# epfl-lts2/pygsp

Hardware: AMD Instinct MI355X
Metric: filtered-vertices/sec (N·Nsig·K/s) + achieved HBM GB/s vs roofline, 1M-vertex K=30 (higher is better)
Workload: dtype f64

## Files before the change

pygsp_amd/csrc/gspx_ctx.hip.h:

```cpp
#pragma once

struct Options {
  int64_t kernel = 0;
  int64_t vec = 0;
  int64_t rows_per_wave = 0;
  int64_t narrow_g_log2 = -1;
  int64_t waves_per_block = 4;
  int64_t calib_mix = 0;
  int64_t graph_launch = 2;
  int64_t tile_gather = 1;
  int64_t tile_workgroups = 0;
  int64_t knn_f32 = 1;
  int64_t tile_pad = 1;
  int64_t tile_min_row = 16;
  int64_t staged_copy = 1;
  int64_t staged_copy_min_mb = 32;
  int64_t copy_threads = 0;
  int64_t tile_regroup = 1;
  int64_t tile_lg = 0;
  int64_t edge_vertex_walk = 1;
  int64_t fuse_input = 1;
  int64_t tile_nt = -1;
  int64_t synthesis = 0;
  int64_t alternate_sweep = 1;
  int64_t xcd_remap = 1;
  int64_t combine = 0;
  int64_t ws_limit_mb = 65536;
  int64_t max_batch = 0;
  int64_t gather_rccl = 1;
  int64_t lds_pad_kb = 0;
  int64_t host_pipeline = 1;
  int64_t host_batch = 0;
  int64_t host_edge = 0;
  int64_t host_threads = 0;
  int64_t streamed_alloc = 1;
};

struct gspx_ctx {
  int device = 0;
  int cu_count = 256;
  hipStream_t stream = nullptr;
  Options opt;
  DevMem ws_t;
  DevMem ws_r;
  DevMem ws_w;
  DevMem io_x, io_y;
  DevMem ws_spec;
  DevMem ws_sq, ws_sqp;
  HostPipe* pipe = nullptr;
  CopyStage* copy = nullptr;
  bool counted = false;
  std::mutex comms_mu;
  std::vector<struct gspx_comm*> comms;
  hipEvent_t ev[4] = {nullptr, nullptr, nullptr, nullptr};
  std::vector<hipEvent_t> ev_pool;
  double timing[5] = {0, 0, 0, 0, 0};
  bool capturing = false;
  std::vector<unsigned char> seen_key;
  std::vector<unsigned char> graph_key;
  hipGraphExec_t graph_exec = nullptr;
};

static std::atomic<int> g_live_ctx[64];

static void replay_reset(gspx_ctx* ctx) {
  if (!ctx) return;
  ctx->seen_key.clear();
  ctx->graph_key.clear();
  if (ctx->graph_exec) {
    (void)hipGraphExecDestroy(ctx->graph_exec);
    ctx->graph_exec = nullptr;
  }
}

static int finish_timed(gspx_ctx* ctx, double* kernel_ms) {
  HIPCHK(hipGetLastError());
  HIPCHK(hipStreamSynchronize(ctx->stream));
  float f = 0;
  HIPCHK(hipEventElapsedTime(&f, ctx->ev[0], ctx->ev[1]));
  if (kernel_ms) *kernel_ms = f;
  return GSPX_OK;
}

struct gspx_buf {
  gspx_ctx* ctx = nullptr;
  DevMem mem;
  int64_t bytes = 0;
};

static std::atomic<uint64_t> g_generation{1};

struct gspx_graph {
  gspx_ctx* ctx = nullptr;
  const uint64_t generation = g_generation.fetch_add(1);
  int64_t N = 0;
  int dtype = GSPX_F64;
  bool from_w = false;
  int64_t nnz_l = 0;
  DevMem lptr, lcol, lval, dw;
  int64_t nnz_int = 0;
  DevMem rptr, rcol, rval, fval, coff;
// ... 88 lines not shown
    delete ctx;
    return set_err(GSPX_ERR_HIP, "hipStreamCreate failed: %s", hipGetErrorString(e));
  }
  for (int i = 0; i < 4; ++i) {
    e = hipEventCreate(&ctx->ev[i]);
    if (e != hipSuccess) {
      delete ctx;
      return set_err(GSPX_ERR_HIP, "hipEventCreate failed: %s", hipGetErrorString(e));
    }
  }
  *out = ctx;
  return GSPX_OK;
}

static void comm_invalidate_all(gspx_ctx* ctx);

extern "C" int gspx_ctx_destroy(gspx_ctx* ctx) {
  replay_reset(ctx);
  if (!ctx) return GSPX_OK;
  if (ctx->counted) g_live_ctx[ctx->device & 63].fetch_sub(1);
  comm_invalidate_all(ctx);
  if (ctx->graph_exec) {
    (void)hipGraphExecDestroy(ctx->graph_exec);
    ctx->graph_exec = nullptr;
  }
  (void)hipSetDevice(ctx->device);
  if (ctx->stream) (void)hipStreamSynchronize(ctx->stream);
  for (int i = 0; i < 4; ++i)
    if (ctx->ev[i]) (void)hipEventDestroy(ctx->ev[i]);
  for (hipEvent_t e : ctx->ev_pool) (void)hipEventDestroy(e);
  ctx->ws_t.release();
  ctx->ws_r.release();
  ctx->ws_w.release();
  ctx->io_x.release();
  ctx->io_y.release();
  ctx->ws_spec.release();
  ctx->ws_sq.release();
  ctx->ws_sqp.release();
  if (ctx->pipe) {
    ctx->pipe->destroy();
    delete ctx->pipe;
    ctx->pipe = nullptr;
  }
  if (ctx->copy) {
    ctx->copy->destroy();
    delete ctx->copy;
    ctx->copy = nullptr;
  }
  if (ctx->stream) (void)hipStreamDestroy(ctx->stream);
  delete ctx;
  return GSPX_OK;
}

extern "C" int gspx_ctx_sync(gspx_ctx* ctx) {
  if (!ctx) return set_err(GSPX_ERR_INVALID, "null ctx");
  HIPCHK(hipSetDevice(ctx->device));
  HIPCHK(hipStreamSynchronize(ctx->stream));
  return GSPX_OK;
}

struct OptionDef {
  const char* key;
  int64_t Options::*slot;
  bool (*ok)(int64_t);
  const char* refusal;
};
static const OptionDef OPTION_TABLE[] = {
    {"kernel", &Options::kernel, [](int64_t v) { return v == 0 || v == 1 || v == 2 || v == 5; },
     "kernel must be 0 (auto), 1 (panel), 2 (narrow) or 5 (LDS-staged)"},
    {"vec", &Options::vec, [](int64_t v) { return v == 0 || v == 1 || v == 2 || v == 4; }, "vec must be 0, 1, 2 or 4"},
    {"rows_per_wave", &Options::rows_per_wave, [](int64_t v) { return v >= 0 && v <= 1024; },
     "rows_per_wave must be in [0, 1024] (0 = auto)"},
    {"narrow_g_log2", &Options::narrow_g_log2, [](int64_t v) { return v >= -1 && v <= 6; },
     "narrow_g_log2 must be in [-1, 6] (-1 = auto)"},
    {"waves_per_block", &Options::waves_per_block, [](int64_t v) { return v == 4 || v == 8 || v == 16; },
     "waves_per_block must be 4, 8 or 16"},
    {"alternate_sweep", &Options::alternate_sweep, nullptr, nullptr},
    {"synthesis", &Options::synthesis, nullptr, nullptr},
    {"tile_gather", &Options::tile_gather, nullptr, nullptr},
    {"graph_launch", &Options::graph_launch, nullptr, nullptr},
    {"tile_workgroups", &Options::tile_workgroups, nullptr, nullptr},
    {"tile_lg", &Options::tile_lg, nullptr, nullptr},
    {"tile_regroup", &Options::tile_regroup, nullptr, nullptr},
    {"staged_copy", &Options::staged_copy, nullptr, nullptr},
    {"staged_copy_min_mb", &Options::staged_copy_min_mb, nullptr, nullptr},
    {"copy_threads", &Options::copy_threads, nullptr, nullptr},
    {"tile_min_row", &Options::tile_min_row, nullptr, nullptr},
    {"tile_pad", &Options::tile_pad, nullptr, nullptr},
    {"knn_f32", &Options::knn_f32, nullptr, nullptr},
    {"tile_nt", &Options::tile_nt, nullptr, nullptr},
    {"fuse_input", &Options::fuse_input, nullptr, nullptr},
    {"edge_vertex_walk", &Options::edge_vertex_walk, nullptr, nullptr},
    {"xcd_remap", &Options::xcd_remap, nullptr, nullptr},
    {"combine", &Options::combine, nullptr, nullptr},
    {"ws_limit_mb", &Options::ws_limit_mb, nullptr, nullptr},
    {"max_batch", &Options::max_batch, nullptr, nullptr},
    {"gather_rccl", &Options::gather_rccl, nullptr, nullptr},
    {"lds_pad_kb", &Options::lds_pad_kb, nullptr, nullptr},
    {"host_pipeline", &Options::host_pipeline, nullptr, nullptr},
    {"host_batch", &Options::host_batch, nullptr, nullptr},
    {"host_edge", &Options::host_edge, nullptr, nullptr},
    {"host_threads", &Options::host_threads, nullptr, nullptr},
    {"streamed_alloc", &Options::streamed_alloc, nullptr, nullptr},
};

static const OptionDef* find_option(const char* key) {
  if (key)
    for (const OptionDef& d : OPTION_TABLE)
      if (!strcmp(key, d.key)) return &d;
  set_err(GSPX_ERR_INVALID, "unknown option '%s'", key ? key : "(null)");
  return nullptr;
}

extern "C" int gspx_ctx_set_option(gspx_ctx* ctx, const char* key, int64_t value) {
  replay_reset(ctx);
  if (!ctx) return set_err(GSPX_ERR_INVALID, "null ctx");
  const OptionDef* d = find_option(key);
  if (!d) return GSPX_ERR_INVALID;
  if (d->ok && !d->ok(value)) return set_err(GSPX_ERR_INVALID, "%s", d->refusal);
  ctx->opt.*d->slot = value;
  if (d->slot == &Options::streamed_alloc) {
    const bool on = value != 0;
    (void)hipSetDevice(ctx->device);
    for (DevMem* m : {&ctx->ws_t, &ctx->ws_r}) {
      if (!on && m->va_size) {
        (void)hipStreamSynchronize(ctx->stream);
        m->release();
      }
      m->streamed = on;
    }
  }
  return GSPX_OK;
}

extern "C" int gspx_ctx_get_option(gspx_ctx* ctx, const char* key, int64_t* value) {
  if (!ctx || !value) return set_err(GSPX_ERR_INVALID, "null argument");
  if (key && !strcmp(key, "retired_va_mb")) {
    *value = (int64_t)(g_retired_va_bytes.load() >> 20);
    return GSPX_OK;
  }
  const OptionDef* d = find_option(key);
  if (!d) return GSPX_ERR_INVALID;
  *value = ctx->opt.*d->slot;
  return GSPX_OK;
}

extern "C" int gspx_buf_alloc(gspx_ctx* ctx, int64_t bytes, gspx_buf** out) {
  if (!ctx || !out || bytes < 0) return set_err(GSPX_ERR_INVALID, "gspx_buf_alloc: bad argument");
  *out = nullptr;
  HIPCHK(hipSetDevice(ctx->device));
  gspx_buf* b = new gspx_buf();
  b->ctx = ctx;
  b->bytes = bytes;
  int rc = b->mem.alloc((size_t)bytes);
  if (rc != GSPX_OK) {
    delete b;
    return rc;
  }
  *out = b;
  return GSPX_OK;
}

extern "C" int gspx_buf_free(gspx_buf* b) {
  if (!b) return GSPX_OK;
  (void)hipSetDevice(b->ctx->device);
  (void)hipStreamSynchronize(b->ctx->stream);
// ... 144 lines not shown
```

pygsp_amd/csrc/gspx_poly.hip.h:

```cpp
#pragma once

struct PlanStep {
  double scale = 1.0, gamma = -1.0;
  int flush = 0;
  int final = 0;
  std::vector<double> w;
};

static void make_plan_fused(int nf, int M, const std::vector<double>& cp, bool acc_existing,
                            bool final_to_y, std::vector<PlanStep>& plan) {
  const int K = M - 1;
  plan.assign((size_t)K, PlanStep());
  int covered = -1;
  bool first = !acc_existing;
  for (int k = 1; k <= K; ++k) {
    PlanStep& st = plan[(size_t)k - 1];
    st.scale = (k == 1) ? 0.5 : 1.0;
    st.gamma = (k == 1) ? 0.0 : -1.0;
    st.w.assign((size_t)nf * 3, 0.0);
    const bool must = (k == K) || (k >= 2 && (k - 2) > covered);
    if (!must) continue;
    st.flush = first ? 1 : 2;
    first = false;
    st.final = (k == K && final_to_y) ? 1 : 0;
// ... 250 lines not shown
}
static size_t sqnorm_parts(const gspx_ctx* ctx, int N, unsigned w) {
  return (size_t)sqnorm_gx(ctx, N, w) * SQ_PASS * w;
}

template <typename T>
static int launch_combine_sqnorm(gspx_ctx* ctx, const T* slots, int nslots, size_t slot_stride, unsigned pitch, int N,
                                 unsigned w, const SqNorms& sq, hipStream_t st) {
  const size_t lds = (size_t)nslots * 64 * sizeof(double);
  const int cwl = sqnorm_cwl(w);
  const dim3 grid((unsigned)sqnorm_gx(ctx, N, w), (w + (1u << cwl) - 1) >> cwl);
  for (int f0 = 0; f0 < sq.nf; f0 += SQ_PASS) {
    const int here = std::min(SQ_PASS, sq.nf - f0);
    const int fb = here <= 8 ? 2 : here <= 32 ? 8 : 32;
    typedef void (*kern_t)(const T*, int, size_t, u32, int, int, int, const double*, int, double*);
    const kern_t kern = fb == 2 ? k_combine_sqnorm<T, 2> : fb == 8 ? k_combine_sqnorm<T, 8> : k_combine_sqnorm<T, 32>;
    if (lds > ((size_t)64 << 10))
      HIPCHK(hipFuncSetAttribute((const void*)kern, hipFuncAttributeMaxDynamicSharedMemorySize, (int)lds));
    hipLaunchKernelGGL(kern, grid, dim3(256), lds, st, slots, nslots, slot_stride, (u32)pitch, N, (int)w, cwl,
                       sq.cf + f0, sq.ldc, sq.part);
    const int64_t n = (int64_t)here * w;
    hipLaunchKernelGGL(k_sqnorm_reduce, dim3((unsigned)((n + 255) / 256)), dim3(256), 0, st, sq.part, (int)grid.x,
                       4 * fb, here, (int)w, sq.out + (size_t)f0 * sq.ldo, sq.ldo);
  }
  return GSPX_OK;
}

template <typename T> static bool tile_geometry(const gspx_graph* g, const Options& opt, unsigned ld) {
  constexpr int TVEC = 16 / (int)sizeof(T);
  const size_t U = (size_t)g->N * ld;
  return opt.tile_gather && g->gt_rows == GSPX_TILE_BR && (size_t)ld * sizeof(T) >= (size_t)opt.tile_min_row &&
         (ld % TVEC) == 0 && U * sizeof(T) < ((size_t)1 << 31) && (size_t)g->nnz_int * sizeof(T) < ((size_t)1 << 31);
}
template <typename T>
static bool tile_usable(const gspx_graph* g, const Options& opt, unsigned ld, const T* y, unsigned ldy) {
  constexpr int TVEC = 16 / (int)sizeof(T);
  return tile_geometry<T>(g, opt, ld) && (ldy % TVEC) == 0 && (((uintptr_t)y / sizeof(T)) % TVEC) == 0;
}
template <typename T>
static int launch_step_tile(gspx_graph* g, const Options& opt, TileArgs<T> t, unsigned ld, hipStream_t st,
                            const T* vals = nullptr) {
  const size_t rowb = (size_t)ld * sizeof(T);
  int lg = rowb <= 16 ? 1 : rowb <= 32 ? 2 : rowb <= 64 ? 4 : rowb <= 128 ? 8 : 16;
  if (opt.tile_lg == 8 || opt.tile_lg == 4 || opt.tile_lg == 2) lg = rowb <= 128 ? std::max(lg, (int)opt.tile_lg) : 16;
  const bool narrow = lg < 16;
  const int ncol = narrow ? 1 : (int)((rowb + 255) / 256);
  const int flavour = t.old_rows ? 1 : t.nin > 0 ? 2 : 0;
  typedef void (*kern_t)(const TileArgs<T>);
  static const kern_t wide[3][3] = {
      {k_step_tile<T, 0>, k_step_tile<T, 1>, k_step_tile<T, 2>},
      {k_step_tile<T, 0, 16, true>, k_step_tile<T, 1, 16, true>, k_step_tile<T, 2, 16, true>},
      {k_step_tile<T, 0, 16, false, true>, k_step_tile<T, 1, 16, false, true>, k_step_tile<T, 2, 16, false, true>}};
  static const kern_t slim[3][4] = {
      {k_step_tile<T, 1, 1, false, false, 64>, k_step_tile<T, 1, 2, false, false, 128>,
       k_step_tile<T, 1, 4, false, false, 256>, k_step_tile<T, 1, 8>},
      {k_step_tile<T, 1, 1, true, false, 64>, k_step_tile<T, 1, 2, true, false, 128>,
       k_step_tile<T, 1, 4, true, false, 256>, k_step_tile<T, 1, 8, true>},
      {k_step_tile<T, 1, 1, false, true, 64>, k_step_tile<T, 1, 2, false, true, 128>,
       k_step_tile<T, 1, 4, false, true, 256>, k_step_tile<T, 1, 8, false, true>}};
  kern_t kern = narrow ? slim[flavour][lg == 1 ? 0 : lg == 2 ? 1 : lg == 4 ? 2 : 3] : wide[flavour][ncol <= 2 ? ncol : 0];
  unsigned threads = narrow ? 64u * (unsigned)lg : 512u;
  bool mix = false;
  if (opt.calib_mix && !narrow && flavour == 0) {
    static const kern_t mixk[2][3] = {
        {k_step_tile<T, 0, 16, false, false, 512, 16, 1>, k_step_tile<T, 1, 16, false, false, 512, 16, 1>,
         k_step_tile<T, 2, 16, false, false, 512, 16, 1>},
        {k_step_tile<T, 0, 16, false, false, 512, 16, 2>, k_step_tile<T, 1, 16, false, false, 512, 16, 2>,
         k_step_tile<T, 2, 16, false, false, 512, 16, 2>}};
    kern = mixk[opt.calib_mix == 2 ? 1 : 0][ncol <= 2 ? ncol : 0];
    mix = true;
  }
  const int pieces = (int)(rowb / 16);
  if (opt.tile_regroup && ncol == 1 && flavour != 1 && pieces < lg && !mix) {
#define GSPX_CL(LG_, CL_, NT_) \
  (flavour == 2 ? (kern_t)k_step_tile<T, 1, LG_, false, true, NT_, CL_> : (kern_t)k_step_tile<T, 1, LG_, false, false, NT_, CL_>)
    kern_t k2 = nullptr;
    unsigned nt2 = 0;
    if (lg == 4 && pieces == 3) k2 = GSPX_CL(4, 3, 192), nt2 = 192;
    else if (lg == 8 && pieces == 5) k2 = GSPX_CL(8, 5, 320), nt2 = 320;
    else if (lg == 16 && pieces == 10) k2 = GSPX_CL(16, 10, 320), nt2 = 320;
#undef GSPX_CL
    if (k2) kern = k2, threads = nt2;
  }
  size_t lds = g->gt_lds;
  if (lg < 8)
    lds = std::min(lds, (size_t)GSPX_TILE_MAXN1 * 16 * lg + (((size_t)g->gt_entmax * sizeof(T) + 15) & ~(size_t)15) +
                            (((size_t)g->gt_entmax + 15) & ~(size_t)15) + 64);
  if (lg < 8) lds = (lds + 2047) & ~(size_t)2047;
  int per_cu = 2;
  {
    struct Known { size_t attr = 0; std::map<size_t, int> fit; };
    static std::map<std::pair<const void*, int>, Known> known;
    static std::mutex lds_mu;
    std::lock_guard<std::mutex> lock(lds_mu);
    Known& k = known[std::make_pair((const void*)kern, g->ctx->device)];
    if (k.attr < lds) {
      HIPCHK(hipFuncSetAttribute((const void*)kern, hipFuncAttributeMaxDynamicSharedMemorySize, (int)lds));
      k.attr = lds;
    }
    if (lg < 8) {
      auto it = k.fit.find(lds);
      if (it == k.fit.end()) {
        int fit = 2;
        HIPCHK(hipOccupancyMaxActiveBlocksPerMultiprocessor(&fit, (const void*)kern, (int)threads, lds));
        it = k.fit.emplace(lds, std::max(2, std::min(fit, 16))).first;
      }
      per_cu = it->second;
    }
  }
  t.rowptr = g->rptr.as<int>();
  t.col = g->rcol.as<int>();
  t.val = vals ? vals : g->fval.as<T>();
  t.hdr = g->gt_hdr.as<int>();
  if (!t.s1rows) t.s1rows = g->gt_s1rows.as<int>();
  t.lidx = g->gt_lidx.as<unsigned char>();
  t.N = (int)g->N;
  t.ld = ld;
  t.panel_bytes = (unsigned)((size_t)g->N * ld * sizeof(T));
  t.val_bytes = (unsigned)((size_t)g->nnz_int * sizeof(T));
  t.lidx_bytes = (unsigned)((size_t)g->nnz_int);
  t.nb = g->gt_nb;
  t.ncol = ncol;
  t.per_xcd = (t.nb + 7) / 8;
  t.lds_bytes = (int)lds;
  unsigned nwg = (unsigned)std::max<int64_t>(8, ((int64_t)per_cu * g->ctx->cu_count) / 8 * 8);
  if (opt.tile_workgroups > 0)
    nwg = (unsigned)std::max<int64_t>(8, std::min<int64_t>(opt.tile_workgroups, 1 << 20) / 8 * 8);
  nwg = std::min(nwg, 8u * (unsigned)std::max(t.per_xcd, 1));
  t.nt = opt.tile_nt >= 0 ? (int)opt.tile_nt : ((size_t)g->N * ld * sizeof(T) >= ((size_t)192 << 20) ? 5 : 0);
  hipLaunchKernelGGL(kern, dim3(nwg), dim3(threads), lds, st, t);
  return GSPX_OK;
}

template <typename T>
static int prepare_coff(gspx_graph* g, const Shape& shape, unsigned ld, hipStream_t st) {
  if (shape.kernel == 5 && g->coff_ldb != ld * (unsigned)sizeof(T)) {
    CHK(g->coff.ensure(((size_t)g->nnz_int + 64) * sizeof(unsigned)));
    const int nb = std::max(1, (int)((g->N + 255) / 256));
    hipLaunchKernelGGL((k_coff<T>), dim3(nb), dim3(256), 0, st, g->rptr.as<int>(), g->rcol.as<int>(), (int)g->N,
                       ld * (unsigned)sizeof(T), g->coff.as<unsigned>());
    g->coff_ldb = ld * (unsigned)sizeof(T);
  }
  return GSPX_OK;
}

template <typename T> static int vec_cap(int v, unsigned ld, const T* p) {
  while (v > 1 && ((ld % v) != 0 || (((uintptr_t)p / sizeof(T)) % v) != 0)) v /= 2;
  return v;
}

struct WorkPanels {
  bool tile_direct, padded;
  unsigned ldw;
};
template <typename T>
static WorkPanels work_panels(const gspx_graph* g, const Options& opt, bool tiles, size_t planes, unsigned ld,
                              const T* y, unsigned ldy) {
  constexpr unsigned TVEC = 16 / (unsigned)sizeof(T);
  const unsigned ldp = (ld + TVEC - 1) / TVEC * TVEC;
  auto window = [&](unsigned w) { return planes * (size_t)g->N * w * sizeof(T) < ((size_t)1 << 31); };
  const bool pad_pays = opt.tile_pad == 2 || ld >= 2 ||
                        (size_t)g->nnz_int * (sizeof(T) + 4) >= ((size_t)20 << 20);
  WorkPanels p;
  p.tile_direct = tiles && tile_usable<T>(g, opt, ld, y, ldy) && window(ld);
  p.padded = !p.tile_direct && tiles && opt.tile_pad && pad_pays && tile_geometry<T>(g, opt, ldp) && window(ldp);
  p.ldw = p.padded ? ldp : ld;
  return p;
}

template <typename T>
static StepArgs<T> step_base(const gspx_graph* g, unsigned ld, T* y, unsigned ldy) {
  StepArgs<T> a{};
  a.rowptr = g->rptr.as<int>();
  a.col = g->rcol.as<int>();
  a.val = g->fval.as<T>();
  a.N = (int)g->N;
  a.ld = ld;
  a.curbytes = (u32)((size_t)g->N * ld * sizeof(T));
  a.y = y;
  a.ldy = ldy;
  a.perm = g->has_perm ? g->perm.as<int>() : nullptr;
  return a;
}

static int batch_events(gspx_ctx* ctx, size_t& ev_idx, hipEvent_t ev[4]) {
  for (int i = 0; i < 4; ++i) ev[i] = pool_event(ctx, ++ev_idx);
  if (!ev[0] || !ev[1] || !ev[2] || !ev[3]) return set_err(GSPX_ERR_HIP, "hipEventCreate failed");
  HIPCHK(hipEventRecord(ev[0], ctx->stream));
  return GSPX_OK;
}

// ... 249 lines not shown
      continue;
    }
    a.wts = ctx->ws_w.as<T>() + (size_t)k * nf;
    a.final = (k == 0) ? 1 : 0;
    a.flush = 0;
    if (k == K) {
      a.cur = S;
      a.old = S;
      a.out = B[k & 1];
      a.scale = T(0);
      a.gamma = T(0);
    } else {
      a.cur = B[(k + 1) & 1];
      a.out = B[k & 1];
      const bool has_b2 = (k + 2 <= K);
      a.old = has_b2 ? B[k & 1] : a.cur;
      a.gamma = has_b2 ? T(-1) : T(0);
      a.scale = (k == 0) ? T(0.5) : T(1);
    }
    a.reverse = (opt.alternate_sweep && (k & 1)) ? 1 : 0;
    launch_step<T>(a, shape, opt, st, g->coff.as<unsigned>());
  }
  HIPCHK(hipEventRecord(ev[2], st));
  if (padded) {
    const unsigned nbp = (unsigned)std::min<size_t>(((size_t)N * ld + 255) / 256, 65536);
    hipLaunchKernelGGL((k_permute_out_pad<T>), dim3(nbp), dim3(256), 0, st, B[0], ldw, y, ldy, ld, N, perm);
  }
  HIPCHK(hipEventRecord(ev[3], st));
  HIPCHK(hipGetLastError());
  return GSPX_OK;
}

template <typename T>
static int run_program_batch(gspx_graph* g, int S, const double* sc, const double* be, const double* ga, bool old_is_x,
                             const T* x, unsigned ldx, T* y, unsigned ldy, unsigned ld, size_t& ev_idx) {
  gspx_ctx* ctx = g->ctx;
  Options opt = ctx->opt;
  hipStream_t st = ctx->stream;
  const int N = (int)g->N;
  const size_t U = (size_t)N * ld;
  const Shape shape = choose_shape(opt, sizeof(T), ld, vec_cap(4, ldy, y));
  const int* perm = g->has_perm ? g->perm.as<int>() : nullptr;

  const T hw[3] = {T(1), T(0), T(0)};
  CHK(ctx->ws_w.ensure(sizeof(hw) + 64));
  HIPCHK(hipMemcpyAsync(ctx->ws_w.p, hw, sizeof(hw), hipMemcpyHostToDevice, st));
  HIPCHK(hipStreamSynchronize(st));
  CHK(ctx->ws_t.ensure((old_is_x ? 3 : 2) * U * sizeof(T) + 256));
  T* X = ctx->ws_t.as<T>();
  T* H[2] = {X + U, old_is_x ? X + 2 * U : X};

  hipEvent_t ev[4];
  CHK(batch_events(ctx, ev_idx, ev));
  launch_permute_in<T>(x, ldx, X, ld, N, perm, vec_cap(shape.vec, ldx, x), st);
  HIPCHK(hipEventRecord(ev[1], st));

  CHK(prepare_coff<T>(g, shape, ld, st));
  StepArgs<T> a = step_base<T>(g, ld, y, ldy);
  a.nf = 1;
  a.racc = H[0];
  a.wts = ctx->ws_w.as<T>();
  const bool tile_ok = tile_usable<T>(g, opt, ld, y, ldy);
  for (int s = 0; s < S; ++s) {
    const bool last = s == S - 1;
    const T* cur = (s == 0) ? X : H[(s - 1) & 1];
    T* out = H[s & 1];
    const T* old = old_is_x ? X : (const T*)out;
    const double gam = (!old_is_x && s == 0) ? 0.0 : ga[s];
    if (tile_ok) {
      TileArgs<T> t{};
      t.cur = cur;
      t.old = gam == 0.0 ? cur : old;
      t.out = out;
      t.racc = H[0];
      t.y = y;
      t.ldy = ldy;
      t.perm = perm;
      t.scale = (T)sc[s];
      t.beta = (T)be[s];
      t.gamma = (T)gam;
      t.flush = 0;
      t.final = last ? 1 : 0;
      t.reverse = (opt.alternate_sweep && (s & 1)) ? 1 : 0;
      CHK(launch_step_tile<T>(g, opt, t, ld, st));
      continue;
    }
    a.cur = cur;
    a.old = gam == 0.0 ? cur : old;
    a.out = out;
    a.scale = (T)sc[s];
    a.beta = (T)be[s];
    a.gamma = (T)gam;
    a.flush = last ? 1 : 0;
    a.final = last ? 1 : 0;
    a.reverse = (opt.alternate_sweep && (s & 1)) ? 1 : 0;
    launch_step<T>(a, shape, opt, st, g->coff.as<unsigned>());
  }
  HIPCHK(hipEventRecord(ev[2], st));
  HIPCHK(hipEventRecord(ev[3], st));
  HIPCHK(hipGetLastError());
  return GSPX_OK;
}

template <typename T>
static int filter_dev_t(gspx_graph* g, double lmax, int Nf, int M, const double* coeffs,
                        int64_t Nsig, const T* x, T* y, int mode) {
  gspx_ctx* ctx = g->ctx;
  const Options& opt = ctx->opt;
  const int64_t N = g->N;
  for (int i = 0; i < 5; ++i) ctx->timing[i] = 0;
  if (N == 0 || Nsig == 0) return GSPX_OK;
  CHK(ensure_factor<T>(g, lmax));
  std::vector<double> cp;
  halve_c0(Nf, M, coeffs, cp);

  const int K = M - 1;
  const bool analysis = mode == GSPX_ANALYSIS;
  bool deferred = analysis && (opt.combine == 2 || (opt.combine == 0 && Nf >= 2));
  const size_t budget = (size_t)std::max<int64_t>(opt.ws_limit_mb, 1) << 20;
  if (deferred && (size_t)N * sizeof(T) * M * (size_t)std::min<int64_t>(Nsig, 4) > budget) deferred = false;
  int64_t max_ld = 0;
  CHK(batch_width(g, sizeof(T), deferred ? (size_t)M : (size_t)(2 + Nf), Nsig, &max_ld));

  std::vector<unsigned char> key;
  const bool graph_mode =
      analysis && Nsig <= max_ld &&
      (opt.graph_launch == 1 || (opt.graph_launch == 2 && (size_t)N * Nsig * sizeof(T) <= ((size_t)32 << 20)));
  if (graph_mode) {
    auto put = [&](const void* p, size_t n) {
      const unsigned char* b = (const unsigned char*)p;
      key.insert(key.end(), b, b + n);
    };
    put(&g->generation, sizeof(g->generation));
    const void* ptrs[] = {x, y, ctx->ws_t.p, ctx->ws_r.p, ctx->ws_w.p, g->coff.p, g->gt_hdr.p, g->gt_s1nat.p,
                          g->fval.p, g->perm.p};
    put(ptrs, sizeof(ptrs));
    put(&lmax, sizeof(lmax));
    put(&g->fval_lmax, sizeof(g->fval_lmax));
    put(&Nf, sizeof(Nf));
    put(&M, sizeof(M));
    put(&Nsig, sizeof(Nsig));
    put(cp.data(), cp.size() * sizeof(double));
    put(&opt, sizeof(opt));
    put(&g->gt_rows, sizeof(g->gt_rows));
    put(&g->gt_slow, sizeof(g->gt_slow));
    if (ctx->graph_exec && !key.empty() && ctx->graph_key == key) {
      HIPCHK(hipEventRecord(ctx->ev[0], ctx->stream));
      HIPCHK(hipGraphLaunch(ctx->graph_exec, ctx->stream));
      HIPCHK(hipEventRecord(ctx->ev[1], ctx->stream));
      HIPCHK(hipStreamSynchronize(ctx->stream));
      float gms = 0;
      HIPCHK(hipEventElapsedTime(&gms, ctx->ev[0], ctx->ev[1]));
      ctx->timing[0] = gms;
      ctx->timing[1] = gms;
      ctx->timing[2] = (double)K;
      return GSPX_OK;
    }
    if (!key.empty() && ctx->seen_key == key) {
      if (ctx->graph_exec) {
        (void)hipGraphExecDestroy(ctx->graph_exec);
        ctx->graph_exec = nullptr;
      }
      hipGraph_t graph = nullptr;
      size_t dummy = 0;
      HIPCHK(hipStreamBeginCapture(ctx->stream, hipStreamCaptureModeThreadLocal));
      ctx->capturing = true;
// ... 297 lines not shown
```

pygsp_amd/csrc/gspx_tile_kernels.hip.h:

```cpp
#pragma once

#include "gspx_kernels.hip.h"

namespace gspx {

template <typename T> struct TileArgs {
  const int* rowptr;
  const int* col;
  const T* val;
  const int* hdr;
  const int* s1rows;
  const u8* lidx;
  const T* cur;
  const T* old;
  const int* old_rows;
  T* out;
  T* racc;
  T* y;
  const int* perm;
  int N;
  u32 ld, ldy;
  u32 panel_bytes, val_bytes, lidx_bytes;
  int nb, ncol, per_xcd;
  int lds_bytes;
  T scale, gamma;
  T beta;
  T wn, wc, wo;
  const T* inp;
  const T* wts;
  int nin;
  int flush;
  int final;
  int reverse;
  int nt;
};

constexpr int GSPX_TILE_BR = 64;
constexpr int GSPX_TILE_MAXN1 = 160;

template <typename T, int NCOL, int LG, bool OLDNAT> struct TileSchedule {
  static constexpr bool PF = !OLDNAT;
  static constexpr bool TILE_LAST = PF && LG == 16;
  static constexpr bool PF_ENTRIES = PF;
  static constexpr bool META_AFTER = !OLDNAT && LG == 16 && NCOL == 0;
};

template <typename T, int NCOL, int LG = 16, bool OLDNAT = false, bool INS = false, int NT = 512, int CL = LG,
          int MIX = 0>
__global__ __launch_bounds__(NT, 4) void k_step_tile(const TileArgs<T> a) {
  static_assert(NT == 512 || (NT == 64 * LG && NCOL == 1) || (CL < LG && NCOL == 1 && NT % 64 == 0 && NT % CL == 0),
                "narrow builds: one row per group, one chunk per row");
  constexpr int BR = GSPX_TILE_BR;
  static_assert(CL <= LG && (BR % (NT / CL)) == 0, "compute groups must tile the block's rows");
  constexpr int MAXN1 = GSPX_TILE_MAXN1;
  constexpr bool PF = TileSchedule<T, NCOL, LG, OLDNAT>::PF;
  constexpr bool META_AFTER = TileSchedule<T, NCOL, LG, OLDNAT>::META_AFTER;
  constexpr bool TILE_LAST = TileSchedule<T, NCOL, LG, OLDNAT>::TILE_LAST;
  constexpr bool PF_ENTRIES = TileSchedule<T, NCOL, LG, OLDNAT>::PF_ENTRIES;
  constexpr int VEC = 16 / (int)sizeof(T);
  typedef typename VT<T, VEC>::t V;
  typedef __attribute__((address_space(3))) void* lds_ptr;
  extern __shared__ __attribute__((aligned(16))) unsigned char gspx_smem[];

  const int tid = threadIdx.x;
  constexpr int NGD = NT / LG;
  constexpr int NG = NT / CL;
  constexpr int NE = (512 + NT - 1) / NT;
  constexpr int RPG = BR / NG;
  constexpr int ST = (MAXN1 + NGD - 1) / NGD;
  constexpr int RB = LG * 16;
  const int lane_d = tid & (LG - 1);
  const int grp_d = tid / LG;
  const int lane16 = CL == LG ? lane_d : tid % CL;
  const int grp = CL == LG ? grp_d : tid / CL;
  const int wave = tid >> 6;
  const int nwx = (int)(gridDim.x >> 3);
  const int xlo = (int)(blockIdx.x & 7) * a.per_xcd;
  int k1 = xlo + a.per_xcd;
  if (k1 > a.nb) k1 = a.nb;
  const int k0 = xlo + (int)(blockIdx.x >> 3);
  if (k0 >= k1) return;

  constexpr u32 POISON = 0x80000000u;
  const rsrc_t rcur = __builtin_amdgcn_make_buffer_rsrc((void*)a.cur, 0, a.panel_bytes, 0x00020000);
  const rsrc_t rold = __builtin_amdgcn_make_buffer_rsrc((void*)a.old, 0, a.panel_bytes, 0x00020000);
  const rsrc_t rra = __builtin_amdgcn_make_buffer_rsrc((void*)a.racc, 0, a.panel_bytes, 0x00020000);
  const rsrc_t rv = __builtin_amdgcn_make_buffer_rsrc((void*)a.val, 0, a.val_bytes, 0x00020000);
  const rsrc_t ri = __builtin_amdgcn_make_buffer_rsrc((void*)a.lidx, 0, a.lidx_bytes, 0x00020000);
  const u32 ldb = a.ld * (u32)sizeof(T);

  struct Meta { int rows[ST]; int rp[RPG + 1]; int orow[OLDNAT ? RPG : 1]; };
  const int xflip = xlo + k1 - 1;
  const bool rev = a.reverse != 0;
  auto phys = [&](int p) { return rev ? xflip - p : p; };
  auto load_hdr = [&](int p) { return *(const int4*)(a.hdr + (size_t)phys(p) * 4); };
  auto uniform = [](int4 h) {
    int4 u;
    u.x = __builtin_amdgcn_readfirstlane(h.x); u.y = __builtin_amdgcn_readfirstlane(h.y);
    u.z = __builtin_amdgcn_readfirstlane(h.z); u.w = __builtin_amdgcn_readfirstlane(h.w);
    return u;
  };
  auto load_meta = [&](int k, const int4& h) {
    Meta m;
    const int n1 = h.y;
#pragma unroll
    for (int t = 0; t < ST; ++t) {
      const int u = grp_d + NGD * t;
      m.rows[t] = a.s1rows[h.x + (u < n1 ? u : 0)];
    }
    int r = phys(k) * BR + grp * RPG;
#pragma unroll
    for (int t = 0; t < RPG + 1; ++t) m.rp[t] = a.rowptr[(r + t) <= a.N ? (r + t) : a.N];
    if constexpr (OLDNAT) {
#pragma unroll
      for (int t = 0; t < RPG; ++t) m.orow[t] = a.old_rows[(r + t) < a.N ? (r + t) : a.N - 1];
    }
    return m;
  };
  V* const tile = (V*)gspx_smem;
  auto stage = [&](const Meta& m, int n1, u32 cb) {
#pragma unroll
    for (int t = 0; t < ST; ++t) {
      if (grp_d + NGD * t < n1)
        __builtin_amdgcn_raw_ptr_buffer_load_lds(rcur, (lds_ptr)(gspx_smem + (wave * (64 / LG) + NGD * t) * RB), 16,
                                                 (u32)m.rows[t] * ldb + cb, 0, 0, 0);
    }
  };
  auto chunk_off_d = [&](int c) {
    const u32 col0 = (c * LG + lane_d) * VEC;
    return col0 < a.ld ? col0 * (u32)sizeof(T) : POISON;
  };
  auto chunk_off = [&](int c) {
    const u32 col0 = (c * LG + lane16) * VEC;
    return col0 < a.ld ? col0 * (u32)sizeof(T) : POISON;
  };

  V ov[RPG], ra[RPG];
  u32x4 ev[NE], ei = 0;
#pragma unroll
  for (int q = 0; q < NE; ++q) ev[q] = 0;
  auto prefetch_rows = [&](const Meta& m, int blk, int c) {
    const int r0 = phys(blk) * BR + grp * RPG;
    const u32 cb = chunk_off(c);
#pragma unroll
    for (int t = 0; t < RPG; ++t) {
      const u32 off = (r0 + t < a.N && cb != POISON) ? (u32)(r0 + t) * ldb + cb : POISON;
      u32 oo = a.gamma != T(0) ? off : POISON;
      if constexpr (OLDNAT) oo = (off != POISON && a.gamma != T(0)) ? (u32)m.orow[t] * ldb + cb : POISON;
      if (a.nt & 4) ov[t] = __builtin_bit_cast(V, __builtin_amdgcn_raw_buffer_load_b128(rold, oo, 0, 2));
      else ov[t] = VT<T, VEC>::bload(rold, oo);
      const u32 ro = a.flush == 2 ? off : POISON;
      if (a.nt & 2) ra[t] = __builtin_bit_cast(V, __builtin_amdgcn_raw_buffer_load_b128(rra, ro, 0, 2));
      else ra[t] = VT<T, VEC>::bload(rra, ro);
    }
  };
  auto prefetch_entries = [&](const int4& h) {
    const int nv16 = (h.w * (int)sizeof(T) + 15) >> 4, ni16 = (h.w + 15) >> 4;
    const u32 io = tid < ni16 ? (u32)h.z + tid * 16u : POISON;
#pragma unroll
    for (int q = 0; q < NE; ++q) {
      const int i = tid + q * NT;
      const u32 vo = i < nv16 ? (u32)h.z * (u32)sizeof(T) + i * 16u : POISON;
      if (a.nt & 1) ev[q] = __builtin_amdgcn_raw_buffer_load_b128(rv, vo, 0, 2);
      else ev[q] = __builtin_amdgcn_raw_buffer_load_b128(rv, vo, 0, 0);
    }
    if (a.nt & 1) ei = __builtin_amdgcn_raw_buffer_load_b128(ri, io, 0, 2);
    else ei = __builtin_amdgcn_raw_buffer_load_b128(ri, io, 0, 0);
  };

  int4 H = uniform(load_hdr(k0));
  Meta M = load_meta(k0, H);
  int k = k0, kn = k0 + nwx, knn = k0 + 2 * nwx;
  int4 Hn = uniform(load_hdr(kn < k1 ? kn : k0));
  if constexpr (!TILE_LAST) {
    if (H.y >= 0) stage(M, H.y, chunk_off_d(0));
  }
  if constexpr (PF) prefetch_rows(M, k0, 0);
  if constexpr (PF_ENTRIES) {
    if (H.y >= 0) prefetch_entries(H);
  }
  if constexpr (TILE_LAST) {
    __builtin_amdgcn_sched_barrier(0);
    if (H.y >= 0) stage(M, H.y, chunk_off_d(0));
    __builtin_amdgcn_sched_barrier(0);
  }

  auto pass = [&](const int c, const bool first, const bool last) __attribute__((always_inline)) {
    const int n1 = H.y, rp0 = H.z, ent = H.w;
    const bool fast = n1 >= 0;
    T* const mval = (T*)(tile + (fast ? n1 : 0) * LG);
    u8* const midx = (u8*)(mval + ent);
    const int row0 = phys(k) * BR + grp * RPG;
    int rs[RPG + 1];
#pragma unroll
    for (int t = 0; t < RPG + 1; ++t) rs[t] = M.rp[t] & ~3;
    const u32 col0 = (c * LG + lane16) * VEC;
    const bool on = col0 < a.ld;
    const u32 cb = on ? col0 * (u32)sizeof(T) : POISON;
    if constexpr (!PF) prefetch_rows(M, k, c);
    V ins[INS ? RPG : 1];
#pragma unroll
    for (int t = 0; t < (INS ? RPG : 1); ++t) ins[t] = 0;
    if constexpr (INS) {
      const rsrc_t rin = __builtin_amdgcn_make_buffer_rsrc((void*)a.inp, 0, a.panel_bytes * (u32)a.nin, 0x00020000);
      for (int f = 0; f < a.nin; ++f) {
        const T w = a.wts[f];
#pragma unroll
        for (int t = 0; t < RPG; ++t) {
          const u32 off = (row0 + t < a.N) ? (u32)(row0 + t) * ldb + cb : POISON;
          ins[t] += w * VT<T, VEC>::bload(rin, off == POISON ? POISON : off + (u32)f * a.panel_bytes);
        }
      }
    }
    if constexpr (!PF_ENTRIES) {
      if (first && fast) prefetch_entries(H);
    }
    int4 Hv = Hn;
    if constexpr (!META_AFTER) {
      if (last) {
        M = load_meta(kn < k1 ? kn : k, Hn);
        Hv = load_hdr(knn < k1 ? knn : k);
      }
    }
    __builtin_amdgcn_sched_barrier(0);
    if (first && fast) {
      const int nv16 = (ent * (int)sizeof(T) + 15) >> 4, ni16 = (ent + 15) >> 4;
#pragma unroll
      for (int q = 0; q < NE; ++q)
        if (tid + q * NT < nv16) *(u32x4*)((unsigned char*)mval + (tid + q * NT) * 16) = ev[q];
      if (tid < ni16) *(u32x4*)((unsigned char*)midx + tid * 16) = ei;
      for (int i = tid + NE * NT; i < nv16; i += NT)
        *(u32x4*)((unsigned char*)mval + i * 16) =
            __builtin_amdgcn_raw_buffer_load_b128(rv, (u32)rp0 * (u32)sizeof(T) + i * 16u, 0, 0);
      for (int i = tid + NT; i < ni16; i += NT)
        *(u32x4*)((unsigned char*)midx + i * 16) =
            __builtin_amdgcn_raw_buffer_load_b128(ri, (u32)rp0 + i * 16u, 0, 0);
    }
    if constexpr (TILE_LAST && !META_AFTER) {
      constexpr int NMETA = ST + RPG + 1 + 1;
      static_assert(NMETA < 16, "vmcnt immediate");
      if (last && !INS) __builtin_amdgcn_s_waitcnt(0x0070 | NMETA);
      else __builtin_amdgcn_s_waitcnt(0x0070);
    } else {
      __builtin_amdgcn_s_waitcnt(0x0070);
    }
    if constexpr (MIX != 2) __syncthreads();
    if constexpr (META_AFTER) {
      if (last) {
        M = load_meta(kn < k1 ? kn : k, Hn);
        Hv = load_hdr(knn < k1 ? knn : k);
      }
    }
    __builtin_amdgcn_sched_barrier(0);
    V nv[RPG], res[RPG];
#pragma unroll
    for (int t = 0; t < RPG; ++t) {
      const int s = rs[t], e = rs[t + 1];
      V acc = 0, self = 0;
      if (MIX && fast) {
        self = tile[(int)midx[s - rp0] * LG + lane16];
        acc = mval[s - rp0] * self;
      } else if (fast) {
        acc = lds_row_dot<T, V, LG, u8>(mval + (s - rp0), midx + (s - rp0), row0 + t < a.N ? e - s : 0, tile, lane16,
                                        self);
      } else if (row0 + t < a.N) {
        for (int j = s; j < e; ++j) {
          const int cc = a.col[j];
          const V xv = VT<T, VEC>::bload(rcur, cc < a.N ? (u32)cc * ldb + cb : POISON);
          if (j == s) self = xv;
          acc += a.val[j] * xv;
        }
      }
      nv[t] = a.scale * acc + a.gamma * ov[t] + a.beta * self;
      if constexpr (INS) nv[t] += ins[t];
      res[t] = a.wn * nv[t] + a.wc * self + a.wo * ov[t];
      if (a.flush == 2) res[t] += ra[t];
    }
    __builtin_amdgcn_s_waitcnt(0xC07F);
    if constexpr (MIX != 2) __builtin_amdgcn_s_barrier();
    bool more = true;
    if (last) {
      const int4 Hnn = uniform(Hv);
      H = Hn;
      Hn = Hnn;
      more = kn < k1;
    }
    __builtin_amdgcn_sched_barrier(0);
    if constexpr (!PF) {
      if (more && H.y >= 0) stage(M, H.y, chunk_off_d(last ? 0 : c + 1));
    }
#pragma unroll
    for (int t = 0; t < RPG; ++t) {
      const int row = row0 + t;
      if (row < a.N && on) {
        if (a.final && !a.flush) {
          const size_t orow = a.perm ? (size_t)a.perm[row] : (size_t)row;
          *(V*)(a.y + orow * a.ldy + col0) = nv[t];
          continue;
        }
        if (a.nt & 8) __builtin_nontemporal_store(nv[t], (V*)(a.out + (size_t)row * a.ld + col0));
        else *(V*)(a.out + (size_t)row * a.ld + col0) = nv[t];
        if (a.flush) {
          if (a.final) {
            const size_t orow = a.perm ? (size_t)a.perm[row] : (size_t)row;
            *(V*)(a.y + orow * a.ldy + col0) = res[t];
          } else {
            if (a.nt & 2) __builtin_nontemporal_store(res[t], (V*)(a.racc + (size_t)row * a.ld + col0));
            else *(V*)(a.racc + (size_t)row * a.ld + col0) = res[t];
          }
        }
      }
    }
    __builtin_amdgcn_sched_barrier(0);
    if constexpr (PF) {
      if (more) {
        const int nc = last ? 0 : c + 1;
        if constexpr (!TILE_LAST) {
          if (H.y >= 0) stage(M, H.y, chunk_off_d(nc));
        }
        prefetch_rows(M, last ? kn : k, nc);
        if constexpr (PF_ENTRIES) {
          if (last && H.y >= 0) prefetch_entries(H);
        }
        if constexpr (TILE_LAST) {
          __builtin_amdgcn_sched_barrier(0);
          if (H.y >= 0) stage(M, H.y, chunk_off_d(nc));
          __builtin_amdgcn_sched_barrier(0);
        }
      }
    }
    if (last) {
      k = kn;
      kn = knn;
      knn += nwx;
    }
    return more;
  };
  for (;;) {
    if constexpr (NCOL == 1) {
      if (!pass(0, true, true)) break;
    } else if constexpr (NCOL == 2) {
      pass(0, true, false);
      if (!pass(1, false, true)) break;
    } else {
      bool more = true;
      for (int c = 0; c < a.ncol; ++c) more = pass(c, c == 0, c == a.ncol - 1);
      if (!more) break;
    }
  }
}

}

namespace gspx {

constexpr int GSPX_TILE_SORTCAP = 4096;
constexpr int GSPX_TILE_TMPCAP = 256;

__global__ __launch_bounds__(256) void k_tiles_unique(const int* __restrict__ rowptr,
                                                      const int* __restrict__ col, int N, int nb,
                                                      int* __restrict__ tmp, int* __restrict__ n1) {
  constexpr int BR = GSPX_TILE_BR;
  __shared__ unsigned keys[GSPX_TILE_SORTCAP];
  __shared__ int wsum[4];
  const int b = blockIdx.x;
  const int r0 = b * BR, r1 = min(r0 + BR, N);
  const int e0 = rowptr[r0] & ~3, e1 = rowptr[r1] & ~3;
  const int ent = e1 - e0;
  if (ent > GSPX_TILE_SORTCAP) {
    if (threadIdx.x == 0) n1[b] = GSPX_TILE_TMPCAP + 1;
    return;
  }
  int n = 1;
  while (n < ent) n <<= 1;
  for (int i = threadIdx.x; i < n; i += 256) {
    unsigned v = 0xFFFFFFFFu;
    if (i < ent) {
      const int c = col[e0 + i];
      if (c < N) v = (unsigned)c;
    }
    keys[i] = v;
  }
  __syncthreads();
  for (int k = 2; k <= n; k <<= 1)
    for (int j = k >> 1; j > 0; j >>= 1) {
      for (int i = threadIdx.x; i < n; i += 256) {
        const int l = i ^ j;
        if (l > i) {
          const unsigned a = keys[i], c = keys[l];
          const bool up = (i & k) == 0;
          if ((a > c) == up) {
// ... 77 lines not shown
```

Before: 187.4 billion.

## Add two-panel tile kernel variant for gamma-zero steps with higher occupancy

Adds a specialised 256-thread tile-step kernel for steps where gamma is zero. It skips loading the old panel and the running accumulator, and drops the flush/res logic. Its launch bounds allow three or more blocks per CU, and it is selected only when the occupancy query confirms at least three fit. The aim is to cut register pressure and memory traffic on those steps to raise occupancy. This costs extra template instantiations, and the variant covers only the first step or other gamma-zero steps.

Measured after the change: 187.7 billion (median of 3 runs). About the same (+0.2%).

```diff
diff --git a/pygsp_amd/csrc/gspx_ctx.hip.h b/pygsp_amd/csrc/gspx_ctx.hip.h
--- a/pygsp_amd/csrc/gspx_ctx.hip.h
+++ b/pygsp_amd/csrc/gspx_ctx.hip.h
@@ -17,6 +17,7 @@
   int64_t staged_copy_min_mb = 32;
   int64_t copy_threads = 0;
   int64_t tile_regroup = 1;
+  int64_t tile_twopanel = 1;
   int64_t tile_lg = 0;
   int64_t edge_vertex_walk = 1;
   int64_t fuse_input = 1;
@@ -271,6 +272,7 @@
     {"tile_workgroups", &Options::tile_workgroups, nullptr, nullptr},
     {"tile_lg", &Options::tile_lg, nullptr, nullptr},
     {"tile_regroup", &Options::tile_regroup, nullptr, nullptr},
+    {"tile_twopanel", &Options::tile_twopanel, nullptr, nullptr},
     {"staged_copy", &Options::staged_copy, nullptr, nullptr},
     {"staged_copy_min_mb", &Options::staged_copy_min_mb, nullptr, nullptr},
     {"copy_threads", &Options::copy_threads, nullptr, nullptr},
diff --git a/pygsp_amd/csrc/gspx_poly.hip.h b/pygsp_amd/csrc/gspx_poly.hip.h
--- a/pygsp_amd/csrc/gspx_poly.hip.h
+++ b/pygsp_amd/csrc/gspx_poly.hip.h
@@ -356,31 +356,51 @@
 #undef GSPX_CL
     if (k2) kern = k2, threads = nt2;
   }
+  kern_t kern3 = nullptr;
+  if (t.twopanel && opt.tile_twopanel && !narrow && flavour == 0 && !mix && threads == 512u) {
+    static const kern_t two[3] = {k_step_tile<T, 0, 16, false, false, 256, 16, 0, 3, true>,
+                                  k_step_tile<T, 1, 16, false, false, 256, 16, 0, 3, true>,
+                                  k_step_tile<T, 2, 16, false, false, 256, 16, 0, 3, true>};
+    kern3 = two[ncol <= 2 ? ncol : 0];
+  }
   size_t lds = g->gt_lds;
   if (lg < 8)
     lds = std::min(lds, (size_t)GSPX_TILE_MAXN1 * 16 * lg + (((size_t)g->gt_entmax * sizeof(T) + 15) & ~(size_t)15) +
                             (((size_t)g->gt_entmax + 15) & ~(size_t)15) + 64);
   if (lg < 8) lds = (lds + 2047) & ~(size_t)2047;
   int per_cu = 2;
-  {
+  auto prepare = [&](kern_t kn, unsigned nthreads, int* fit_out) -> int {
     struct Known { size_t attr = 0; std::map<size_t, int> fit; };
     static std::map<std::pair<const void*, int>, Known> known;
     static std::mutex lds_mu;
     std::lock_guard<std::mutex> lock(lds_mu);
-    Known& k = known[std::make_pair((const void*)kern, g->ctx->device)];
+    Known& k = known[std::make_pair((const void*)kn, g->ctx->device)];
     if (k.attr < lds) {
-      HIPCHK(hipFuncSetAttribute((const void*)kern, hipFuncAttributeMaxDynamicSharedMemorySize, (int)lds));
+      HIPCHK(hipFuncSetAttribute((const void*)kn, hipFuncAttributeMaxDynamicSharedMemorySize, (int)lds));
       k.attr = lds;
     }
-    if (lg < 8) {
+    if (fit_out) {
       auto it = k.fit.find(lds);
       if (it == k.fit.end()) {
         int fit = 2;
-        HIPCHK(hipOccupancyMaxActiveBlocksPerMultiprocessor(&fit, (const void*)kern, (int)threads, lds));
-        it = k.fit.emplace(lds, std::max(2, std::min(fit, 16))).first;
+        HIPCHK(hipOccupancyMaxActiveBlocksPerMultiprocessor(&fit, (const void*)kn, (int)nthreads, lds));
+        it = k.fit.emplace(lds, fit).first;
       }
-      per_cu = it->second;
-    }
+      *fit_out = it->second;
+    }
+    return GSPX_OK;
+  };
+  if (kern3) {
+    int fit = 0;
+    CHK(prepare(kern3, 256u, &fit));
+    if (fit >= 3) kern = kern3, threads = 256u, per_cu = 3;
+  }
+  if (kern != kern3 && lg < 8) {
+    int fit = 2;
+    CHK(prepare(kern, threads, &fit));
+    per_cu = std::max(2, std::min(fit, 16));
+  } else if (kern != kern3) {
+    CHK(prepare(kern, threads, nullptr));
   }
   t.rowptr = g->rptr.as<int>();
   t.col = g->rcol.as<int>();
@@ -796,6 +816,7 @@
       t.flush = 0;
       t.final = last ? 1 : 0;
       t.reverse = (opt.alternate_sweep && (s & 1)) ? 1 : 0;
+      t.twopanel = gam == 0.0 ? 1 : 0;
       CHK(launch_step_tile<T>(g, opt, t, ld, st));
       continue;
     }
diff --git a/pygsp_amd/csrc/gspx_tile_kernels.hip.h b/pygsp_amd/csrc/gspx_tile_kernels.hip.h
--- a/pygsp_amd/csrc/gspx_tile_kernels.hip.h
+++ b/pygsp_amd/csrc/gspx_tile_kernels.hip.h
@@ -33,30 +33,34 @@
   int final;
   int reverse;
   int nt;
+  int twopanel;
 };
 
 constexpr int GSPX_TILE_BR = 64;
 constexpr int GSPX_TILE_MAXN1 = 160;
 
-template <typename T, int NCOL, int LG, bool OLDNAT> struct TileSchedule {
+template <typename T, int NCOL, int LG, bool OLDNAT, bool TWO = false> struct TileSchedule {
   static constexpr bool PF = !OLDNAT;
   static constexpr bool TILE_LAST = PF && LG == 16;
   static constexpr bool PF_ENTRIES = PF;
-  static constexpr bool META_AFTER = !OLDNAT && LG == 16 && NCOL == 0;
+  static constexpr bool META_AFTER = !OLDNAT && LG == 16 && (NCOL == 0 || TWO);
 };
 
 template <typename T, int NCOL, int LG = 16, bool OLDNAT = false, bool INS = false, int NT = 512, int CL = LG,
-          int MIX = 0>
-__global__ __launch_bounds__(NT, 4) void k_step_tile(const TileArgs<T> a) {
-  static_assert(NT == 512 || (NT == 64 * LG && NCOL == 1) || (CL < LG && NCOL == 1 && NT % 64 == 0 && NT % CL == 0),
-                "narrow builds: one row per group, one chunk per row");
+          int MIX = 0, int WPS = 4, bool TWO = false>
+__global__ __launch_bounds__(NT, WPS) void k_step_tile(const TileArgs<T> a) {
+  static_assert(NT == 512 || (NT == 64 * LG && NCOL == 1) || (CL < LG && NCOL == 1 && NT % 64 == 0 && NT % CL == 0) ||
+                    (TWO && NT == 256 && LG == 16 && CL == LG),
+                "narrow builds: one row per group, one chunk per row; two-panel build: 256 threads, four rows per group");
+  static_assert(!TWO || (!OLDNAT && !INS && !MIX), "two-panel build: no third panel of any kind");
   constexpr int BR = GSPX_TILE_BR;
   static_assert(CL <= LG && (BR % (NT / CL)) == 0, "compute groups must tile the block's rows");
   constexpr int MAXN1 = GSPX_TILE_MAXN1;
-  constexpr bool PF = TileSchedule<T, NCOL, LG, OLDNAT>::PF;
-  constexpr bool META_AFTER = TileSchedule<T, NCOL, LG, OLDNAT>::META_AFTER;
-  constexpr bool TILE_LAST = TileSchedule<T, NCOL, LG, OLDNAT>::TILE_LAST;
-  constexpr bool PF_ENTRIES = TileSchedule<T, NCOL, LG, OLDNAT>::PF_ENTRIES;
+  typedef TileSchedule<T, NCOL, LG, OLDNAT, TWO> Sched;
+  constexpr bool PF = Sched::PF;
+  constexpr bool META_AFTER = Sched::META_AFTER;
+  constexpr bool TILE_LAST = Sched::TILE_LAST;
+  constexpr bool PF_ENTRIES = Sched::PF_ENTRIES;
   constexpr int VEC = 16 / (int)sizeof(T);
   typedef typename VT<T, VEC>::t V;
   typedef __attribute__((address_space(3))) void* lds_ptr;
@@ -135,11 +139,12 @@
     return col0 < a.ld ? col0 * (u32)sizeof(T) : POISON;
   };
 
-  V ov[RPG], ra[RPG];
+  V ov[TWO ? 1 : RPG], ra[TWO ? 1 : RPG];
   u32x4 ev[NE], ei = 0;
 #pragma unroll
   for (int q = 0; q < NE; ++q) ev[q] = 0;
   auto prefetch_rows = [&](const Meta& m, int blk, int c) {
+    if constexpr (TWO) return;
     const int r0 = phys(blk) * BR + grp * RPG;
     const u32 cb = chunk_off(c);
 #pragma unroll
@@ -252,7 +257,7 @@
       }
     }
     __builtin_amdgcn_sched_barrier(0);
-    V nv[RPG], res[RPG];
+    V nv[RPG], res[TWO ? 1 : RPG];
 #pragma unroll
     for (int t = 0; t < RPG; ++t) {
       const int s = rs[t], e = rs[t + 1];
@@ -271,10 +276,14 @@
           acc += a.val[j] * xv;
         }
       }
-      nv[t] = a.scale * acc + a.gamma * ov[t] + a.beta * self;
+      V old = 0;
+      if constexpr (!TWO) old = ov[t];
+      nv[t] = a.scale * acc + a.gamma * old + a.beta * self;
       if constexpr (INS) nv[t] += ins[t];
-      res[t] = a.wn * nv[t] + a.wc * self + a.wo * ov[t];
-      if (a.flush == 2) res[t] += ra[t];
+      if constexpr (!TWO) {
+        res[t] = a.wn * nv[t] + a.wc * self + a.wo * old;
+        if (a.flush == 2) res[t] += ra[t];
+      }
     }
     __builtin_amdgcn_s_waitcnt(0xC07F);
     if constexpr (MIX != 2) __builtin_amdgcn_s_barrier();
@@ -293,20 +302,22 @@
     for (int t = 0; t < RPG; ++t) {
       const int row = row0 + t;
       if (row < a.N && on) {
-        if (a.final && !a.flush) {
+        if (a.final && (TWO || !a.flush)) {
           const size_t orow = a.perm ? (size_t)a.perm[row] : (size_t)row;
           *(V*)(a.y + orow * a.ldy + col0) = nv[t];
           continue;
         }
         if (a.nt & 8) __builtin_nontemporal_store(nv[t], (V*)(a.out + (size_t)row * a.ld + col0));
         else *(V*)(a.out + (size_t)row * a.ld + col0) = nv[t];
-        if (a.flush) {
-          if (a.final) {
-            const size_t orow = a.perm ? (size_t)a.perm[row] : (size_t)row;
-            *(V*)(a.y + orow * a.ldy + col0) = res[t];
-          } else {
-            if (a.nt & 2) __builtin_nontemporal_store(res[t], (V*)(a.racc + (size_t)row * a.ld + col0));
-            else *(V*)(a.racc + (size_t)row * a.ld + col0) = res[t];
+        if constexpr (!TWO) {
+          if (a.flush) {
+            if (a.final) {
+              const size_t orow = a.perm ? (size_t)a.perm[row] : (size_t)row;
+              *(V*)(a.y + orow * a.ldy + col0) = res[t];
+            } else {
+              if (a.nt & 2) __builtin_nontemporal_store(res[t], (V*)(a.racc + (size_t)row * a.ld + col0));
+              else *(V*)(a.racc + (size_t)row * a.ld + col0) = res[t];
+            }
           }
         }
       }
```
